# Shibodd/volume_path_tracer

Hardware: AMD Instinct MI355X
Metric: Msamples/s (whole node) + achieved HBM GB/s, wdas_cloud 1920×1080 (higher is better)
Workload: dtype f32

## Files before the change

### __graft_entry__.py

```python
from __future__ import annotations

import subprocess
import sys
from pathlib import Path

ROOT = Path(__file__).resolve().parent


def build() -> None:
    sys.path.insert(0, str(ROOT))
    from volume_path_tracer_amd import build as B

    B.build(verbose=True)
    subprocess.run(["make", "-s", "-C", str(ROOT / "oracle")], check=True)
    subprocess.run(["make", "-s", "-C", str(ROOT / "tests" / "native")], check=True)
    subprocess.run([sys.executable, "-B", "-c", "import sys; sys.path[:0] = [%r, %r]; import alpha_lib, denoise_lib, "
                    "dense_pool_lib; alpha_lib.build_lib(); denoise_lib.build_lib(); dense_pool_lib.build_program()"
                    % (str(ROOT), str(ROOT / "tests"))], check=True)
    import volume_path_tracer_amd
    from volume_path_tracer_amd import capi

    capi.lib()


def smoke() -> None:
    sys.path.insert(0, str(ROOT))
    sys.path.insert(0, str(ROOT / "tests"))
    import numpy as np
    import torch

    import oracle_lib as O
    from volume_path_tracer_amd.render import Integrator
# ... 24 lines not shown
```

### include/vpt_gpu.h

```cpp
#ifndef VPT_GPU_H
#define VPT_GPU_H

#include <stddef.h>
#include <stdint.h>

#ifdef __cplusplus
extern "C" {
#endif

#define VPT_ABI_VERSION 1

enum {
  VPT_OK = 0,
  VPT_E_INVALID = 1,
  VPT_E_HIP = 2,
  VPT_E_IO = 3,
  VPT_E_PARSE = 4,
  VPT_E_NOMEM = 5,
  VPT_E_STATE = 6
};


typedef struct vpt_camera_params {
  float position[3];
// ... 202 lines not shown
  int32_t active;
  float maximum;
} vpt_dda_row;
int vpt_dda_trace(const vpt_grid_desc* density, const float origin[3], const float direction[3], vpt_dda_row* rows,
                  int max_rows, int* n_rows);

int vpt_gpu_majorant_trace(vpt_gpu_ctx* ctx, const float origin[3], const float direction[3],
                           float* rows_host, int max_rows, int* n_rows);

enum { VPT_RNG_REFERENCE = 0, VPT_RNG_PIXEL = 1 };
int vpt_gpu_set_rng_mode(vpt_gpu_ctx* ctx, int mode);
int vpt_gpu_set_pixel_chunk(vpt_gpu_ctx* ctx, int chunk);

int vpt_gpu_set_run_skipping(vpt_gpu_ctx* ctx, int mode);
int vpt_gpu_kernel_variant(const vpt_gpu_ctx* ctx, int* has_temperature, int* run_skipping);

enum {
  VPT_ORDER_JID = 0,
  VPT_ORDER_COST_WAVE_MAJOR = 1,
  VPT_ORDER_COST_TILE_MAJOR = 2,
  VPT_ORDER_COST_TAIL = 3,
  VPT_ORDER_COST_SAME_TILE = 4
};
int vpt_gpu_set_job_order(vpt_gpu_ctx* ctx, int mode);
int vpt_gpu_set_job_order_tail(vpt_gpu_ctx* ctx, int waves);
int vpt_gpu_tile_costs(vpt_gpu_ctx* ctx, float* cost_T, uint32_t* rank_T);
int vpt_gpu_set_tile_costs(vpt_gpu_ctx* ctx, const float* cost_T);
int vpt_gpu_set_job_permutation(vpt_gpu_ctx* ctx, const uint32_t* perm, uint64_t n);

int vpt_gpu_sync(vpt_gpu_ctx* ctx);
// ... 57 lines not shown
```

### volume_path_tracer_amd/capi.py

```python
from __future__ import annotations

import ctypes as C
import os
from pathlib import Path

import numpy as np

PKG_DIR = Path(__file__).resolve().parent
LIB_DIR = PKG_DIR / "lib"
LIB_PATH = Path(os.environ["VPT_LIB"]) if os.environ.get("VPT_LIB") else LIB_DIR / "libvpt_amd.so"

VPT_OK = 0
VPT_BLACKBODY_ROWS = 500


class CameraParams(C.Structure):
    _fields_ = [("position", C.c_float * 3), ("look", C.c_float * 3), ("up", C.c_float * 3),
                ("vfov_deg", C.c_float), ("imaging_ratio", C.c_float)]


class WorkerParams(C.Structure):
    _fields_ = [("single_pixel_enabled", C.c_int32), ("use_jitter", C.c_int32),
                ("single_pixel_coord", C.c_int64 * 2),
                ("infinite_light_xyz", C.c_float * 3), ("infinite_light_multiplier", C.c_float),
# ... 256 lines not shown
    L.vpt_synth_grid.argtypes = [C.c_int, C.c_int]
    L.vpt_synth_grid.restype = gridp
    L.vpt_synth_free.argtypes = [gridp]
    L.vpt_grid_from_nanovdb.argtypes = [C.c_void_p, C.c_size_t, C.POINTER(gridp)]
    L.vpt_grid_read_nvdb.argtypes = [C.c_char_p, C.c_char_p, C.POINTER(gridp)]
    L.vpt_grid_free.argtypes = [gridp]
    L.vpt_film_to_srgb8.argtypes = [fp, C.c_int64, C.c_int64, C.POINTER(C.c_uint8)]
    L.vpt_gpu_trace_jobs.argtypes = [vp, C.c_uint64, C.c_uint64, vp, vp, C.c_uint64, C.POINTER(C.c_uint64), vp]
    L.vpt_gpu_majorant_trace.argtypes = [vp, fp, fp, fp, C.c_int, C.POINTER(C.c_int)]
    L.vpt_dda_trace.argtypes = [C.POINTER(GridDesc), fp, fp, vp, C.c_int, C.POINTER(C.c_int)]
    L.vpt_gpu_set_rng_mode.argtypes = [vp, C.c_int]
    if hasattr(L, "vpt_gpu_set_pixel_chunk"):
        L.vpt_gpu_set_pixel_chunk.argtypes = [vp, C.c_int]
    L.vpt_gpu_set_run_skipping.argtypes = [vp, C.c_int]
    L.vpt_gpu_kernel_variant.argtypes = [vp, C.POINTER(C.c_int), C.POINTER(C.c_int)]
    if hasattr(L, "vpt_gpu_set_film_order"):
        L.vpt_gpu_set_film_order.argtypes = [vp, C.c_int, C.c_uint64]
        L.vpt_gpu_film_order_info.argtypes = [vp, C.POINTER(C.c_int), C.POINTER(C.c_uint64),
                                              C.POINTER(C.c_uint64), C.POINTER(C.c_uint64)]
    if hasattr(L, "vpt_gpu_set_pool_layout"):
        L.vpt_gpu_set_pool_layout.argtypes = [vp, C.c_int]
        L.vpt_gpu_set_pool_cap.argtypes = [vp, C.c_uint64]
        L.vpt_gpu_pool_info.argtypes = [vp, C.POINTER(C.c_int), C.POINTER(C.c_int), C.POINTER(C.c_uint64),
                                        C.POINTER(C.c_uint64), C.POINTER(C.c_double)]
        L.vpt_gpu_debug_read_pool.argtypes = [vp, C.c_int, C.c_uint64, C.c_uint64, fp]
    L.vpt_gpu_set_job_order.argtypes = [vp, C.c_int]
    L.vpt_gpu_set_job_order_tail.argtypes = [vp, C.c_int]
    L.vpt_gpu_tile_costs.argtypes = [vp, fp, C.POINTER(C.c_uint32)]
    L.vpt_gpu_set_tile_costs.argtypes = [vp, fp]
    L.vpt_gpu_set_job_permutation.argtypes = [vp, C.POINTER(C.c_uint32), C.c_uint64]
# ... 63 lines not shown
```

### volume_path_tracer_amd/csrc/vpt_ctx.h

```cpp
#pragma once

#include <hip/hip_runtime.h>

#include <atomic>
#include <chrono>
#include <cstdint>
#include <mutex>
#include <string>
#include <vector>

#include "vpt_internal.h"
#include "vpt_launch.h"

#define VPT_HIP(call)                                                                                 \
  do {                                                                                                \
    hipError_t e_ = (call);                                                                           \
    if (e_ != hipSuccess)                                                                             \
      return ::vpt::set_error(VPT_E_HIP, std::string(#call " failed: ") + hipGetErrorString(e_));            \
  } while (0)

#ifndef VPT_DEFAULT_JOB_ORDER
#define VPT_DEFAULT_JOB_ORDER VPT_ORDER_COST_SAME_TILE
#endif

// ... 51 lines not shown
  uint64_t film_count = 0;
  unsigned long long* job_counter = nullptr;
  hipEvent_t slot_done[64] = {};
  bool slot_used[64] = {};
  uint32_t next_slot = 0;
  std::mutex slot_mu;
  unsigned long long* counters = nullptr;
  unsigned long long* prof = nullptr;
  vpt::DevScene* scene_dev = nullptr;
  vpt::DevScene* scene_lat_dev = nullptr;
  int lat_gate[4] = {1, 65, 1, 1};
  int lat_wave_lanes = 0;
  vpt::DevScene* scene_full_dev = nullptr;
  int full_gate[4] = {0, 0, 0, 0};
  int last_gate_set = -1;
  hipStream_t stream = nullptr;
  bool use_runs = false;
  int pixel_chunk = 0;
  int grid_blocks = 0;
  int cus = 1;
  bool grid_user = false;
  int order_mode = VPT_DEFAULT_JOB_ORDER;
  int order_tail_waves = 0;
  uint32_t* order = nullptr;
  std::vector<float> tile_cost;
  uint32_t* perm = nullptr;
  uint64_t perm_n = 0;
  std::vector<uint32_t> tile_rank;
  float* staging = nullptr;
  std::vector<vpt_gpu_feed*> feed_pool;
// ... 82 lines not shown
```

### volume_path_tracer_amd/csrc/vpt_gpu.hip

```cpp
#include <hip/hip_runtime.h>
#include <pthread.h>
#include <sched.h>
#include <unistd.h>

#include <algorithm>
#include <cmath>
#include <cstdio>
#include <cstdlib>
#include <cstring>
#include <fstream>
#include <functional>
#include <memory>
#include <atomic>
#include <mutex>
#include <chrono>
#include <string>
#include <thread>
#include <vector>

#include "vpt_ctx.h"
#include "vpt_kernels.h"
#include "vpt_denoise.h"

namespace vpt {
// ... 553 lines not shown
  } else if (feed) {
    auto kernel = temp ? vpt::vpt_integrate_kernel<true, false, false, false, false, true>
                       : ctx->use_runs ? vpt::vpt_integrate_kernel<false, false, true, false, false, true>
                                       : vpt::vpt_integrate_kernel<false, false, false, false, false, true>;
    hipLaunchKernelGGL(kernel, dim3(blocks), dim3(vpt::kBlockThreads), 0, s, env, scene, ctx->counters);
  } else {
    auto kernel = temp ? (dbg ? vpt::vpt_integrate_kernel<true, true, false> : vpt::vpt_integrate_kernel<true, false, false>)
                       : ctx->use_runs
                           ? (dbg ? vpt::vpt_integrate_kernel<false, true, true> : vpt::vpt_integrate_kernel<false, false, true>)
                           : (dbg ? vpt::vpt_integrate_kernel<false, true, false> : vpt::vpt_integrate_kernel<false, false, false>);
    if (!dbg && scene == ctx->scene_dev) scene = ctx->scene_full_dev;
    hipLaunchKernelGGL(kernel, dim3(blocks), dim3(vpt::kBlockThreads), 0, s, env, scene, ctx->counters);
  }
  ctx->last_gate_set = scene == ctx->scene_full_dev ? VPT_GATES_FULL
                       : scene == ctx->scene_lat_dev ? VPT_GATES_LATENCY : VPT_GATES_CONTEXT;
  VPT_HIP(hipGetLastError());
  const uint64_t npix = (uint64_t)ctx->scene.W * (uint64_t)ctx->scene.H;
  if (band) {
    const uint32_t chunks = (ctx->scene.tile_area + 63u) / 64u;
    const uint32_t* const list = band->list ? ctx->list_dev : nullptr;
    hipLaunchKernelGGL(ctx->m2 ? vpt::vpt_band_order_kernel<true> : vpt::vpt_band_order_kernel<false>,
                       dim3(band->tiles * chunks), dim3(64), 0, s, ctx->scene_dev, env.film, (const float*)samples,
                       band->tile_lo, band->waves, env.band_groups, band->group, list, ctx->m2);
    VPT_HIP(hipGetLastError());
    VPT_HIP(hipEventRecord(ctx->samples_done, s));
    ctx->samples_used = true;
  } else if (samples) {
    const uint64_t threads = ctx->scene.T * (uint64_t)ctx->scene.tile_area;
    hipLaunchKernelGGL(ctx->m2 ? vpt::vpt_film_order_kernel<true> : vpt::vpt_film_order_kernel<false>,
                       dim3((unsigned)((threads + 255) / 256)), dim3(256), 0, s, ctx->scene_dev, env.film,
// ... 646 lines not shown
  env.gang_target = p->target_error;
  env.gang_floor = p->abs_floor;
  env.gang_min = p->min_waves;
  env.gang_step = p->step_waves;
  env.gang_max = p->max_waves;
  uint32_t slot = 0;
  if ((rc = take_slot(ctx, s, slot))) return rc;
  env.job_counter = ctx->job_counter + 2 * slot;
  env.event_count = ctx->job_counter + 2 * slot + 1;
  const bool temp = ctx->scene.has_temperature != 0;
  auto kernel = temp ? vpt::vpt_integrate_kernel<true, false, false, false, false, false, false, true>
                     : ctx->use_runs ? vpt::vpt_integrate_kernel<false, false, true, false, false, false, false, true>
                                     : vpt::vpt_integrate_kernel<false, false, false, false, false, false, false, true>;
  hipLaunchKernelGGL(kernel, dim3(blocks), dim3(vpt::kBlockThreads), 0, s, env, ctx->scene_full_dev, ctx->counters);
  ctx->last_gate_set = VPT_GATES_FULL;
  VPT_HIP(hipGetLastError());
  ++ctx->ordered_launches;
  VPT_HIP(hipMemcpyAsync(waves_T_host, ctx->gang_waves, (size_t)T * sizeof(uint32_t), hipMemcpyDeviceToHost, s));
  VPT_HIP(hipMemcpyAsync(err_T_host, ctx->tile_err, (size_t)T * sizeof(float), hipMemcpyDeviceToHost, s));
  if ((rc = release_slot(ctx, s, slot))) return rc;
  VPT_HIP(hipStreamSynchronize(s));
  vpt_adaptive_result res{};
  res.jobs_uniform = (uint64_t)p->max_waves * T;
  uint32_t longest = p->min_waves;
  for (uint32_t t = 0; t < T; ++t) {
    res.jobs_rendered += waves_T_host[t];
    longest = std::max(longest, waves_T_host[t]);
    if (waves_T_host[t] >= p->max_waves) ++res.tiles_at_max;
    res.max_error = std::max(res.max_error, err_T_host[t]);
  }
// ... 68 lines not shown
  return VPT_OK;
}

int vpt_gpu_set_run_skipping(vpt_gpu_ctx* ctx, int mode) {
  if (!ctx || mode < -1 || mode > 1) return vpt::set_error(VPT_E_INVALID, "vpt_gpu_set_run_skipping: bad argument");
  if (mode == 1 && ctx->scene.has_temperature)
    return vpt::set_error(VPT_E_INVALID, "vpt_gpu_set_run_skipping: no run-skipping variant with a temperature grid");
  ctx->use_runs = mode < 0 ? (!ctx->scene.has_temperature && ctx->density.run_fraction >= VPT_RUNS_MIN_FRACTION) : mode == 1;
  return VPT_OK;
}

int vpt_gpu_kernel_variant(const vpt_gpu_ctx* ctx, int* has_temperature, int* run_skipping) {
  if (!ctx) return vpt::set_error(VPT_E_INVALID, "null context");
  if (has_temperature) *has_temperature = ctx->scene.has_temperature ? 1 : 0;
  if (run_skipping) *run_skipping = ctx->use_runs ? 1 : 0;
  return VPT_OK;
}

int vpt_gpu_set_pool_layout(vpt_gpu_ctx* ctx, int layout) {
  if (!ctx || layout < VPT_POOL_SPARSE || layout > VPT_POOL_AUTO)
    return vpt::set_error(VPT_E_INVALID, "vpt_gpu_set_pool_layout: bad argument");
  if (ctx->open_feeds.load() > 0) return vpt::set_error(VPT_E_STATE, "vpt_gpu_set_pool_layout: a feed of this context is open");
  if (ctx->frame_waves) return vpt::set_error(VPT_E_STATE, "vpt_gpu_set_pool_layout: a frame is open");
  int rc = ctx_device(ctx);
  if (rc) return rc;
  if ((rc = wait_ctx(ctx))) return rc;
  VPT_HIP(hipDeviceSynchronize());
  ctx->pool_policy = layout;
  rc = apply_pool_layout(ctx, layout);
  const int prc = push_scene(ctx);
// ... 459 lines not shown
```

### volume_path_tracer_amd/csrc/vpt_integrator.h

```cpp
#pragma once

#include <hip/hip_runtime.h>
#include <stdint.h>

#include "vpt_math.h"

namespace vpt {

struct RootTileDev {
  int32_t origin[3];
  float value;
  int32_t active;
  int32_t pad[3];
};

struct DevGrid {
  float mat[9], inv_mat[9], vec[3];
  float background;
  int32_t bbox_min[3], bbox_max[3];
  int32_t r8_org[3], r8_n[3];
  int32_t w8_org[3], w8_n[3];
  uint32_t w8_max;
  int32_t r128_org[3], r128_n[3];
  int32_t root_count, leaf_count;
// ... 141 lines not shown
    }
  }
}

__host__ __device__ __forceinline__ void dense_square(const DevGrid& g, int32_t a, int32_t b, int32_t c, int32_t s,
                                                      float out[4]) {
  const int32_t x = s % 9, yz = s / 9;
  const int32_t i = g.r8_org[0] + a * 8 + x, j = g.r8_org[1] + b * 8 + (yz >> 3), k = g.r8_org[2] + c * 8 + (yz & 7);
  out[0] = value_at(g, i, j, k);
  out[1] = value_at(g, i, j, k + 1);
  out[2] = value_at(g, i, j + 1, k);
  out[3] = value_at(g, i, j + 1, k + 1);
}

__host__ __device__ __forceinline__ float lerpf(float a, float b, float w) { return a + w * (b - a); }
__host__ __device__ __forceinline__ bool trilinear(const DevGrid& g, StencilCell& last, float x, float y, float z,
                                                   float& out) {
  float fi = floorf(x), fj = floorf(y), fk = floorf(z);
  float u = x - fi, v = y - fj, w = z - fk;
  int32_t i = (int32_t)fi, j = (int32_t)fj, k = (int32_t)fk;
  bool refresh = i != last.i || j != last.j || k != last.k;
  if (g.dense) {
    const int32_t a = (i - g.r8_org[0]) >> 3, b = (j - g.r8_org[1]) >> 3, c = (k - g.r8_org[2]) >> 3;
    if ((uint32_t)a < (uint32_t)g.r8_n[0] && (uint32_t)b < (uint32_t)g.r8_n[1] && (uint32_t)c < (uint32_t)g.r8_n[2]) {
      const float4* p = reinterpret_cast<const float4*>(g.dense + dense_index(mad_index(a, b, c, g.r8_n), i, j, k));
      const float4 lo = p[0], hi = p[1];
      last.i = i;
      last.j = j;
      last.k = k;
      last.code = -1;
// ... 185 lines not shown
#endif
  return q / rw;
}

enum : int32_t {
  ST_FETCH = 0,
  ST_PIXEL = 1,
  ST_RAY = 2,
  ST_SAMPLE = 3,
  ST_NEE_DONE = 4,
  ST_FINISH = 5,
  ST_DONE = 6,
  ST_SHADOW = 7,
  ST_FINISH_T = 8
};
enum : int32_t { SM_NEED_SEG = 0, SM_STEP = 1, SM_DRAW = 2, SM_EVAL = 3, SM_NONE = 4 };
enum : int32_t {
  PB_ITER = 0, PB_FETCH, PB_PIXEL, PB_RAY, PB_SAMPLE, PB_NEED_SEG, PB_STEP, PB_DRAW, PB_TRILINEAR,
  PB_EVENT, PB_SHADOW_HIT, PB_NONE, PB_NEE_DONE, PB_FINISH,
  PB_W_WALK, PB_W_EVAL, PB_W_NEE, PB_W_FIN, PB_W_RAY, PB_W_PIX, PB_W_DONE, PB_COUNT
};
enum : int32_t { PT_FETCH = 0, PT_PIXEL, PT_RAY, PT_WALK, PT_EVAL, PT_NEE, PT_FINISH, PT_SEG, PT_STEP, PT_DRAW, PT_COUNT };

enum : int32_t {
  CNT_SAMPLES = 0, CNT_DDA_STEPS, CNT_SEGMENTS, CNT_DRAWS, CNT_STENCILS, CNT_DENSITY_EVALS, CNT_TEMP_STENCILS,
  CNT_SCATTERS, CNT_SHADOW_RAYS, CNT_RNG_DRAWS, CNT_EXCHANGED, CNT_COUNT
};

struct LaneCold {
  int32_t x0, y0, pix;
  uint32_t depth;
// ... 390 lines not shown
      for (int i = 0; i < 3; ++i) lc.ro[i] = cp[i];
      if (S.li_zero) {
        lc.Tr = -1.0f;
        ln.state = ST_NEE_DONE;
      } else {
        lc.Tr = local_const(1.0f);
        ln.shadow = 1;
        ln.state = ST_SHADOW;
      }
    }
  }
  if (Debug && ev == 0) env.event(ln, VPT_EV_NULL, nullptr, nullptr, 0.0f);
  if (ev != 0) ln.sm = SM_NONE;
}

template <bool HasTemp, bool Debug, class Env>
__host__ __device__ __forceinline__ void eval_collision(ScenePtr sp, const DevScene& S, const DevGrid& G, Lane& ln, Env& env) {
  LaneCold& lc = env.cold();
  const float sigma_maj = ln.s_dmaj * S.sigma_t;
  {
    const float dt_m = -math::logf_glibc_unit(lc.y_draw, env.logf_table()) / sigma_maj;
    const float tc = ln.s_t0 + math::div_by_recip(dt_m, ln.scale, ln.rscale);
    if (!(tc < ln.s_t1)) {
      ln.sm = SM_NEED_SEG;
      return;
    }
    ln.s_t0 = tc;
  }
  env.prof(PB_TRILINEAR);
  const float t = ln.s_t0;
  float pi_x = ln.e[0] + ln.d[0] * t, pi_y = ln.e[1] + ln.d[1] * t, pi_z = ln.e[2] + ln.d[2] * t;
  float dens;
  if (Debug) env.tally(CNT_DENSITY_EVALS, 1);
  env.tally(CNT_STENCILS, trilinear(G, lc.dens_cell, pi_x, pi_y, pi_z, dens) ? 1 : 0);
  ln.sm = SM_DRAW;
  if (dens > 0.0f) {
    if (!HasTemp) {
      const bool sh = ln.shadow != 0;
      const float sigma_n = fmaxf(0.0f, sigma_maj - S.sigma_t * dens);
      const float q1 = (sh ? sigma_n : S.sigma_a * dens) / sigma_maj;
      const float tr = lc.Tr * q1;
      const bool draw = !sh || tr <= 0.05f;
      float u = 0.0f;
      if (draw) {
        u = rng_uniform(ln.rng);
        if (Debug) env.tally(CNT_RNG_DRAWS, 1);
      }
      if (!sh) {
        primary_event<HasTemp, Debug>(sp, S, G, ln, lc, env, pi_x, pi_y, pi_z, dens, q1, (S.sigma_s * dens) / sigma_maj, u);
// ... 82 lines not shown
  ln.scale = ln.rscale = ln.maj = ln.Tn = ln.T1 = ln.s_t0 = ln.s_t1 = ln.s_dmaj = 0.0f;
  ln.dim = 0;
  ln.pw = 0;
}

template <class Env, class = void>
struct env_is_gang {
  static constexpr bool value = false;
};
template <class Env>
struct env_is_gang<Env, decltype((void)Env::kGang)> {
  static constexpr bool value = Env::kGang;
};


template <bool HasTemp, bool Debug, bool Runs, class Env>
__host__ __device__ __forceinline__ void lane_iteration(ScenePtr sp, Lane& ln, Env& env) {
  env.prof(PB_ITER);
  LaneCold& lc = env.cold();
  int32_t gate_min;
  bool starving;
  {
    const DevScene S = *opaque(sp);
    gate_min = S.gate_min;
    const int32_t n_walking = env.count(ln.state == ST_SAMPLE && ln.sm != SM_EVAL);
    starving = n_walking < S.gate_idle;
  }
  auto go = [&](int32_t st) -> bool {
    const int32_t n = env.count(ln.state == st);
    return n > 0 && (starving || n >= gate_min) && ln.state == st;
  };
  auto go2 = [&](int32_t st_a, int32_t st_b) -> bool {
    const bool mine = ln.state == st_a || ln.state == st_b;
    const int32_t n = env.count(mine);
    return n > 0 && (starving || n >= gate_min) && mine;
  };

  {
    const DevScene S = *opaque(sp);
    const DevGrid& G = S.density;
    (void)G;
    if (go(ST_NEE_DONE)) {
      env.prof(PB_NEE_DONE);
      if (lc.Tr >= 0.0f) {
        float c = lc.rd[0] * S.wi[0] + (lc.rd[1] * S.wi[1] + lc.rd[2] * S.wi[2]);
        float p = hg_eval(S, c);
        float pt = p * lc.Tr;
        lc.L[0] = lc.L[0] + pt * S.Li[0];
        lc.L[1] = lc.L[1] + pt * S.Li[1];
        lc.L[2] = lc.L[2] + pt * S.Li[2];
      } else {
        lc.L[0] = lc.L[0] == 0.0f ? 0.0f : lc.L[0];
        lc.L[1] = lc.L[1] == 0.0f ? 0.0f : lc.L[1];
        lc.L[2] = lc.L[2] == 0.0f ? 0.0f : lc.L[2];
      }
      float u0 = rng_uniform(ln.rng);
      float u1 = rng_uniform(ln.rng);
      if (Debug) env.tally(CNT_RNG_DRAWS, 2);
      float nd[3];
      sample_hg(S, lc.rd, u0, u1, nd);
      for (int i = 0; i < 3; ++i) lc.rd[i] = nd[i];
      if (Debug) env.event(ln, VPT_EV_SCATTER, lc.ro, lc.rd, 0.0f);
      ++lc.depth;
      ln.shadow = 0;
      ln.state = ST_RAY;
    }
  }
  env.tick(PT_NEE);
  {
    const DevScene S = *opaque(sp);
    const DevGrid& G = S.density;
    (void)G;
    const bool fin = go2(ST_FINISH, ST_FINISH_T);
    if (fin) {
      env.prof(PB_FINISH);
      if (ln.state == ST_FINISH) {
        lc.L[0] = lc.L[0] + S.le_inf[0];
        lc.L[1] = lc.L[1] + S.le_inf[1];
        lc.L[2] = lc.L[2] + S.le_inf[2];
      }
      const int32_t rw = min(S.W - lc.x0, S.tw);
      const int32_t q = (lc.pix & kPixelMask) - 1, y = div_pix(q, rw);
      env.film_add(S, ln, lc.x0 + (q - y * rw), lc.y0 + y, rw);
// ... 134 lines not shown
        dv[1] = math::div_by_recip(dv[1], s, rs);
        dv[2] = math::div_by_recip(dv[2], s, rs);
      }
      for (int i = 0; i < 3; ++i) {
        lc.ro[i] = S.cam_pos[i];
        lc.rd[i] = dv[i];
        lc.L[i] = 0.0f;
      }
      lc.depth = 0;
      ln.shadow = 0;
      ln.state = ST_RAY;
      if (Debug) env.event(ln, VPT_EV_NEW_RAY, lc.ro, lc.rd, 0.0f);
    }
  }
  env.tick(PT_PIXEL);
  {
    const DevScene S = *opaque(sp);
    const DevGrid& G = S.density;
    (void)G;
    if (go2(ST_RAY, ST_SHADOW)) {
      env.prof(PB_RAY);
      const bool primary = ln.state == ST_RAY;
      if (primary && !(lc.depth < S.max_depth)) {
        ln.state = ST_FINISH;
      } else {
        RayDir rd;
        if (primary) {
          rd = ray_dir_setup(G, lc.rd);
        } else {
          for (int i = 0; i < 3; ++i) {
// ... 81 lines not shown
        } else {
          lc.y_draw = y;
          ln.sm = SM_EVAL;
        }
      }
      env.tick(PT_DRAW);
#if VPT_WALK_UNROLL > 1
      }
#endif
      } while (S.gate_walk > 0 && env.count(ln.state == ST_SAMPLE && ln.sm != SM_EVAL) >= S.gate_walk &&
               env.count(ln.state == ST_SAMPLE && ln.sm == SM_EVAL) < S.gate_eval);
      wave_priority(0);
    }
  }
  env.tick(PT_WALK);
  {
    const DevScene S = *opaque(sp);
    const DevGrid& G = S.density;
    (void)G;
    const int32_t n_eval = env.count(ln.state == ST_SAMPLE && ln.sm == SM_EVAL);
    const bool run_eval = n_eval > 0 && (n_eval >= S.gate_eval || env.count(ln.state == ST_SAMPLE && ln.sm != SM_EVAL) < S.gate_idle);
    if (!HasTemp && run_eval) wave_priority(kPrioEval);
    if (run_eval && ln.state == ST_SAMPLE && ln.sm == SM_EVAL) eval_collision<HasTemp, Debug>(sp, S, G, ln, env);
    if (!HasTemp) wave_priority(0);
  }
  env.tick(PT_EVAL);
}

__host__ __device__ __forceinline__ void lane_init(Lane& ln) {
  ln.state = ST_FETCH;
  ln.sm = SM_NONE;
// ... 13 lines not shown
```

### volume_path_tracer_amd/csrc/vpt_kernels.h

```cpp
#pragma once

#include <hip/hip_runtime.h>

#include "vpt_alpha.h"
#include "vpt_internal.h"
#include "vpt_launch.h"

namespace vpt {

constexpr int kCounterCount = CNT_COUNT;
#ifndef VPT_WAVES_FAST
#define VPT_WAVES_FAST 7
#endif
#ifndef VPT_WAVES_SLOW
#define VPT_WAVES_SLOW 4
#endif
#ifndef VPT_WAVES_TEMP
#define VPT_WAVES_TEMP 6
#endif
#ifndef VPT_WAVES_LAT
#define VPT_WAVES_LAT 4
#endif

__shared__ LaneCold g_lane_cold[kBlockThreads];
// ... 45 lines not shown
  uint32_t* gang_waves;
  float* gang_err;
  float gang_target, gang_floor;
  uint32_t gang_min, gang_step, gang_max;
};
typedef const __attribute__((address_space(4))) KernelArgs* ArgsPtr;
__shared__ unsigned long long g_wg_counters[kCounterCount];
#if defined(VPT_PROFILE) || defined(VPT_PROFILE_TIME)
__shared__ unsigned long long g_wg_prof[PT_COUNT + kBlockThreads / 64];
#endif
__shared__ float g_bb_lds[kBbFloats];
__shared__ uint32_t g_film_rank[kBlockThreads];
__shared__ uint32_t g_gang[kBlockThreads / 64][4];
constexpr uint32_t kGangMaxArea = 256;

template <bool RegCold, bool Feed = false, bool Band = false, bool Gang = false>
struct KernelEnvT {
  static_assert(!(RegCold && Feed), "feeds run the throughput kernels only");
  static_assert(!(Band && Feed), "band launches are no feeds");
  static_assert(!(Gang && (RegCold || Feed || Band)), "gang launches run the plain throughput kernels only");
  static constexpr bool kGang = Gang;
  __device__ __forceinline__ ArgsPtr args() const {
    ArgsPtr p = (ArgsPtr)__builtin_amdgcn_kernarg_segment_ptr();
    asm volatile("" : "+s"(p));
    return p;
  }

  __device__ __forceinline__ void tally(int32_t k, int32_t w) {
    const unsigned long long m = __builtin_amdgcn_ballot_w64(w != 0);
    if (m && __lane_id() == (uint32_t)__builtin_ctzll(m))
      atomicAdd(g_wg_counters + k, (unsigned long long)(__popcll(m) * (uint64_t)(w ? w : 1)));
  }

  __device__ __forceinline__ void prof(int32_t id) {
#ifdef VPT_PROFILE
    const unsigned long long m = __ballot(1);
// ... 498 lines not shown
#pragma unroll
      for (int q = 0; q < kXWords / 4; ++q) {
        const uint4 v = g_xchg[q * kBlockThreads + threadIdx.x];
        x[4 * q] = v.x;
        x[4 * q + 1] = v.y;
        x[4 * q + 2] = v.z;
        x[4 * q + 3] = v.w;
      }
      xchg_unpack<HasTemp>(ln, lc, x);
      env.tally(CNT_EXCHANGED, 1);
    }
    __syncthreads();
  }
}

template <bool HasTemp, bool Debug, bool Runs, bool Lat = false, bool Compact = false, bool Feed = false, bool Band = false,
          bool Gang = false>
__global__ __launch_bounds__(kBlockThreads, Compact ? 2 : (Lat ? VPT_WAVES_LAT : (Debug ? VPT_WAVES_SLOW : (HasTemp ? VPT_WAVES_TEMP : VPT_WAVES_FAST)))) void vpt_integrate_kernel(KernelArgs args, const DevScene* scene,
                                                                       unsigned long long* counters) {
  (void)args;
  if (threadIdx.x < kCounterCount) g_wg_counters[threadIdx.x] = 0;
  if (threadIdx.x < 32) g_logf_tab[threadIdx.x >> 1][threadIdx.x & 1] = math::kLogfTab[threadIdx.x >> 1][threadIdx.x & 1];
  if (HasTemp) {
    const float* bb = scene->bb;
    for (int i = threadIdx.x; i < kBbFloats; i += kBlockThreads) g_bb_lds[i] = bb[i];
  }
  __syncthreads();
#if defined(VPT_PROFILE) || defined(VPT_PROFILE_TIME)
  if (threadIdx.x < PT_COUNT) g_wg_prof[threadIdx.x] = 0;
  __syncthreads();
  if (threadIdx.x % 64 == 0) g_wg_prof[PT_COUNT + threadIdx.x / 64] = clock64();
#endif
  static_assert(!(Band && Debug), "band launches have no records or events");
  static_assert(!(Gang && (Debug || Lat || Compact || Feed || Band)), "gang launches run the plain throughput kernels only");
  if constexpr (Gang) {
    if (threadIdx.x < kBlockThreads / 64) {
      g_gang[threadIdx.x][0] = 0xffffffffu;
      g_gang[threadIdx.x][3] = 0;
    }
    __syncthreads();
  }
  KernelEnvT<Lat, Feed, Band, Gang> env;
  env.reg_cold = nullptr;
  Lane ln;
  lane_init(ln);
  LaneCold lc_reg;
  if constexpr (Lat) env.reg_cold = &lc_reg;
  cold_init(env.cold());
  const ScenePtr sp = (ScenePtr)scene;
  if constexpr (Compact) {
    static_assert(Lat && !Debug, "compaction runs in the latency kernel only");
    compact_loop<HasTemp, Runs>(sp, ln, lc_reg, env);
  } else
  while (ln.state != ST_DONE) {
    lane_iteration<HasTemp, Debug, Runs>(sp, ln, env);
    if (Feed &&
        __builtin_amdgcn_ballot_w64(ln.state == ST_FETCH && (env.cold().pix == kFeedPending ||
// ... 411 lines not shown
```

### volume_path_tracer_amd/render.py

```python
from __future__ import annotations

import ctypes as C
import threading
import time
from typing import Optional

import numpy as np

from . import capi


def ceildiv(a: int, b: int) -> int:
    return a // b + (a % b != 0)


class TileProvider:

    def __init__(self, img_size, waves: int, tile_size):
        self.img_w, self.img_h = int(img_size[0]), int(img_size[1])
        self.tile_w, self.tile_h = int(tile_size[0]), int(tile_size[1])
        self.ntx, self.nty = ceildiv(self.img_w, self.tile_w), ceildiv(self.img_h, self.tile_h)
        self.num_tiles = self.ntx * self.nty
        self.requested_waves = int(waves)
        self.max_wave_idx = 0
# ... 267 lines not shown

    def set_run_skipping(self, mode: int) -> None:
        capi.check(capi.lib().vpt_gpu_set_run_skipping(self.h, int(mode)), "vpt_gpu_set_run_skipping")

    def set_latency_kernel(self, mode: int, ungated: int = -1) -> None:
        capi.check(capi.lib().vpt_gpu_set_latency_kernel(self.h, int(mode), int(ungated)), "vpt_gpu_set_latency_kernel")

    def set_compaction(self, every: int) -> None:
        capi.check(capi.lib().vpt_gpu_set_compaction(self.h, int(every)), "vpt_gpu_set_compaction")

    def latency_kernel_info(self) -> dict:
        m, b = C.c_int(), C.c_int()
        capi.check(capi.lib().vpt_gpu_latency_kernel_info(self.h, C.byref(m), C.byref(b)), "vpt_gpu_latency_kernel_info")
        return {"mode": int(m.value), "resident_blocks_per_cu": int(b.value)}

    def kernel_variant(self) -> dict:
        t, r = C.c_int(), C.c_int()
        capi.check(capi.lib().vpt_gpu_kernel_variant(self.h, C.byref(t), C.byref(r)), "vpt_gpu_kernel_variant")
        return {"has_temperature": bool(t.value), "run_skipping": bool(r.value)}

    def set_film_order(self, mode: int, max_bytes: int = 0) -> None:
        capi.check(capi.lib().vpt_gpu_set_film_order(self.h, int(mode), int(max_bytes)), "vpt_gpu_set_film_order")

    def film_order_info(self) -> dict:
        m, b, o, a = C.c_int(), C.c_uint64(), C.c_uint64(), C.c_uint64()
        capi.check(capi.lib().vpt_gpu_film_order_info(self.h, C.byref(m), C.byref(b), C.byref(o), C.byref(a)),
                   "vpt_gpu_film_order_info")
        return {"mode": int(m.value), "buffer_bytes": int(b.value), "ordered_launches": int(o.value),
                "atomic_launches": int(a.value)}

    def set_pool_layout(self, layout: int, cap_bytes: int | None = None) -> None:
        if cap_bytes is not None:
            capi.check(capi.lib().vpt_gpu_set_pool_cap(self.h, int(cap_bytes)), "vpt_gpu_set_pool_cap")
        capi.check(capi.lib().vpt_gpu_set_pool_layout(self.h, int(layout)), "vpt_gpu_set_pool_layout")
# ... 208 lines not shown
```

Baseline: 1712.

## Split density evaluation into issue and finish phases to hide stencil load latency

In the throughput kernels without temperature, density evaluation is split in two. The first phase, at the top of each lane iteration, draws the collision distance and issues the dense 8-voxel stencil loads as two float4 reads. The second phase, after the pixel and fetch stages, does the trilinear interpolation and the event. Moving the NEE-done and later eval blocks lets the memory latency overlap with other state-machine work in the same iteration. The cost is extra live registers across the iteration (two float4s), new sub-states, and a different ordering of work between lanes, which could affect occupancy.

```diff
diff --git a/__graft_entry__.py b/__graft_entry__.py
--- a/__graft_entry__.py
+++ b/__graft_entry__.py
@@ -15,7 +15,8 @@
     subprocess.run(["make", "-s", "-C", str(ROOT / "oracle")], check=True)
     subprocess.run(["make", "-s", "-C", str(ROOT / "tests" / "native")], check=True)
     subprocess.run([sys.executable, "-B", "-c", "import sys; sys.path[:0] = [%r, %r]; import alpha_lib, denoise_lib, "
-                    "dense_pool_lib; alpha_lib.build_lib(); denoise_lib.build_lib(); dense_pool_lib.build_program()"
+                    "dense_pool_lib, eval_split_lib; alpha_lib.build_lib(); denoise_lib.build_lib(); "
+                    "dense_pool_lib.build_program(); eval_split_lib.build_lib()"
                     % (str(ROOT), str(ROOT / "tests"))], check=True)
     import volume_path_tracer_amd
     from volume_path_tracer_amd import capi
diff --git a/include/vpt_gpu.h b/include/vpt_gpu.h
--- a/include/vpt_gpu.h
+++ b/include/vpt_gpu.h
@@ -240,6 +240,7 @@
 
 int vpt_gpu_set_run_skipping(vpt_gpu_ctx* ctx, int mode);
 int vpt_gpu_kernel_variant(const vpt_gpu_ctx* ctx, int* has_temperature, int* run_skipping);
+int vpt_gpu_last_launch_variant(const vpt_gpu_ctx* ctx, int* eval_split);
 
 enum {
   VPT_ORDER_JID = 0,
diff --git a/volume_path_tracer_amd/capi.py b/volume_path_tracer_amd/capi.py
--- a/volume_path_tracer_amd/capi.py
+++ b/volume_path_tracer_amd/capi.py
@@ -294,6 +294,8 @@
         L.vpt_gpu_set_pixel_chunk.argtypes = [vp, C.c_int]
     L.vpt_gpu_set_run_skipping.argtypes = [vp, C.c_int]
     L.vpt_gpu_kernel_variant.argtypes = [vp, C.POINTER(C.c_int), C.POINTER(C.c_int)]
+    if hasattr(L, "vpt_gpu_last_launch_variant"):
+        L.vpt_gpu_last_launch_variant.argtypes = [vp, C.POINTER(C.c_int)]
     if hasattr(L, "vpt_gpu_set_film_order"):
         L.vpt_gpu_set_film_order.argtypes = [vp, C.c_int, C.c_uint64]
         L.vpt_gpu_film_order_info.argtypes = [vp, C.POINTER(C.c_int), C.POINTER(C.c_uint64),
diff --git a/volume_path_tracer_amd/csrc/vpt_ctx.h b/volume_path_tracer_amd/csrc/vpt_ctx.h
--- a/volume_path_tracer_amd/csrc/vpt_ctx.h
+++ b/volume_path_tracer_amd/csrc/vpt_ctx.h
@@ -89,6 +89,7 @@
   vpt::DevScene* scene_full_dev = nullptr;
   int full_gate[4] = {0, 0, 0, 0};
   int last_gate_set = -1;
+  int last_eval_split = -1;
   hipStream_t stream = nullptr;
   bool use_runs = false;
   int pixel_chunk = 0;
diff --git a/volume_path_tracer_amd/csrc/vpt_gpu.hip b/volume_path_tracer_amd/csrc/vpt_gpu.hip
--- a/volume_path_tracer_amd/csrc/vpt_gpu.hip
+++ b/volume_path_tracer_amd/csrc/vpt_gpu.hip
@@ -591,6 +591,7 @@
   }
   ctx->last_gate_set = scene == ctx->scene_full_dev ? VPT_GATES_FULL
                        : scene == ctx->scene_lat_dev ? VPT_GATES_LATENCY : VPT_GATES_CONTEXT;
+  ctx->last_eval_split = vpt::kernel_eval_split(temp, dbg, use_lat) ? 1 : 0;
   VPT_HIP(hipGetLastError());
   const uint64_t npix = (uint64_t)ctx->scene.W * (uint64_t)ctx->scene.H;
   if (band) {
@@ -1267,6 +1268,7 @@
                                      : vpt::vpt_integrate_kernel<false, false, false, false, false, false, false, true>;
   hipLaunchKernelGGL(kernel, dim3(blocks), dim3(vpt::kBlockThreads), 0, s, env, ctx->scene_full_dev, ctx->counters);
   ctx->last_gate_set = VPT_GATES_FULL;
+  ctx->last_eval_split = vpt::kernel_eval_split(temp, false, false) ? 1 : 0;
   VPT_HIP(hipGetLastError());
   ++ctx->ordered_launches;
   VPT_HIP(hipMemcpyAsync(waves_T_host, ctx->gang_waves, (size_t)T * sizeof(uint32_t), hipMemcpyDeviceToHost, s));
@@ -1365,6 +1367,12 @@
   if (!ctx) return vpt::set_error(VPT_E_INVALID, "null context");
   if (has_temperature) *has_temperature = ctx->scene.has_temperature ? 1 : 0;
   if (run_skipping) *run_skipping = ctx->use_runs ? 1 : 0;
+  return VPT_OK;
+}
+
+int vpt_gpu_last_launch_variant(const vpt_gpu_ctx* ctx, int* eval_split) {
+  if (!ctx) return vpt::set_error(VPT_E_INVALID, "null context");
+  if (eval_split) *eval_split = ctx->last_eval_split;
   return VPT_OK;
 }
 
diff --git a/volume_path_tracer_amd/csrc/vpt_integrator.h b/volume_path_tracer_amd/csrc/vpt_integrator.h
--- a/volume_path_tracer_amd/csrc/vpt_integrator.h
+++ b/volume_path_tracer_amd/csrc/vpt_integrator.h
@@ -179,6 +179,31 @@
 }
 
 __host__ __device__ __forceinline__ float lerpf(float a, float b, float w) { return a + w * (b - a); }
+__host__ __device__ __forceinline__ const float4* dense_stencil(const DevGrid& g, int32_t i, int32_t j, int32_t k) {
+  if (g.dense) {
+    const int32_t a = (i - g.r8_org[0]) >> 3, b = (j - g.r8_org[1]) >> 3, c = (k - g.r8_org[2]) >> 3;
+    if ((uint32_t)a < (uint32_t)g.r8_n[0] && (uint32_t)b < (uint32_t)g.r8_n[1] && (uint32_t)c < (uint32_t)g.r8_n[2])
+      return reinterpret_cast<const float4*>(g.dense + dense_index(mad_index(a, b, c, g.r8_n), i, j, k));
+  }
+  return nullptr;
+}
+__host__ __device__ __forceinline__ void lookup_stencil(const DevGrid& g, StencilCell& last, int32_t i, int32_t j, int32_t k,
+                                                        float s[8]) {
+  const int32_t dx = (i ^ last.i) | (j ^ last.j) | (k ^ last.k);
+  const bool same_leaf = last.code >= 0 && dx >= 0 && dx < 8;
+  Cell c;
+  if (same_leaf) {
+    c.code = last.code;
+    c.value = 0.0f;
+  } else {
+    c = cell_at(g, i, j, k);
+  }
+  last.i = i;
+  last.j = j;
+  last.k = k;
+  last.code = c.code;
+  fetch_stencil(g, c, i, j, k, s);
+}
 __host__ __device__ __forceinline__ bool trilinear(const DevGrid& g, StencilCell& last, float x, float y, float z,
                                                    float& out) {
   float fi = floorf(x), fj = floorf(y), fk = floorf(z);
@@ -394,7 +419,7 @@
   ST_SHADOW = 7,
   ST_FINISH_T = 8
 };
-enum : int32_t { SM_NEED_SEG = 0, SM_STEP = 1, SM_DRAW = 2, SM_EVAL = 3, SM_NONE = 4 };
+enum : int32_t { SM_NEED_SEG = 0, SM_STEP = 1, SM_DRAW = 2, SM_EVAL = 3, SM_NONE = 4, SM_FETCHED = 5, SM_FETCHED_LOOKUP = 6 };
 enum : int32_t {
   PB_ITER = 0, PB_FETCH, PB_PIXEL, PB_RAY, PB_SAMPLE, PB_NEED_SEG, PB_STEP, PB_DRAW, PB_TRILINEAR,
   PB_EVENT, PB_SHADOW_HIT, PB_NONE, PB_NEE_DONE, PB_FINISH,
@@ -815,25 +840,90 @@
   if (ev != 0) ln.sm = SM_NONE;
 }
 
+template <class Env>
+__host__ __device__ __forceinline__ bool eval_distance(Lane& ln, const LaneCold& lc, Env& env, float sigma_maj) {
+  const float dt_m = -math::logf_glibc_unit(lc.y_draw, env.logf_table()) / sigma_maj;
+  const float tc = ln.s_t0 + math::div_by_recip(dt_m, ln.scale, ln.rscale);
+  if (!(tc < ln.s_t1)) {
+    ln.sm = SM_NEED_SEG;
+    return false;
+  }
+  ln.s_t0 = tc;
+  return true;
+}
+
+template <bool HasTemp, bool Debug, class Env>
+__host__ __device__ __forceinline__ void eval_event(ScenePtr sp, const DevScene& S, const DevGrid& G, Lane& ln, LaneCold& lc, Env& env,
+                                                    float sigma_maj, float pi_x, float pi_y, float pi_z, float dens);
+
 template <bool HasTemp, bool Debug, class Env>
 __host__ __device__ __forceinline__ void eval_collision(ScenePtr sp, const DevScene& S, const DevGrid& G, Lane& ln, Env& env) {
   LaneCold& lc = env.cold();
   const float sigma_maj = ln.s_dmaj * S.sigma_t;
-  {
-    const float dt_m = -math::logf_glibc_unit(lc.y_draw, env.logf_table()) / sigma_maj;
-    const float tc = ln.s_t0 + math::div_by_recip(dt_m, ln.scale, ln.rscale);
-    if (!(tc < ln.s_t1)) {
-      ln.sm = SM_NEED_SEG;
-      return;
-    }
-    ln.s_t0 = tc;
-  }
+  if (!eval_distance(ln, lc, env, sigma_maj)) return;
   env.prof(PB_TRILINEAR);
   const float t = ln.s_t0;
   float pi_x = ln.e[0] + ln.d[0] * t, pi_y = ln.e[1] + ln.d[1] * t, pi_z = ln.e[2] + ln.d[2] * t;
   float dens;
   if (Debug) env.tally(CNT_DENSITY_EVALS, 1);
   env.tally(CNT_STENCILS, trilinear(G, lc.dens_cell, pi_x, pi_y, pi_z, dens) ? 1 : 0);
+  eval_event<HasTemp, Debug>(sp, S, G, ln, lc, env, sigma_maj, pi_x, pi_y, pi_z, dens);
+}
+
+template <bool Debug, class Env>
+__host__ __device__ __forceinline__ void eval_issue(const DevScene& S, const DevGrid& G, Lane& ln, Env& env, float4& lo, float4& hi) {
+  LaneCold& lc = env.cold();
+  if (!eval_distance(ln, lc, env, ln.s_dmaj * S.sigma_t)) return;
+  env.prof(PB_TRILINEAR);
+  const float t = ln.s_t0;
+  const float pi_x = ln.e[0] + ln.d[0] * t, pi_y = ln.e[1] + ln.d[1] * t, pi_z = ln.e[2] + ln.d[2] * t;
+  const int32_t i = (int32_t)floorf(pi_x), j = (int32_t)floorf(pi_y), k = (int32_t)floorf(pi_z);
+  if (Debug) env.tally(CNT_DENSITY_EVALS, 1);
+  ln.sm = SM_FETCHED_LOOKUP;
+  if (const float4* p = dense_stencil(G, i, j, k)) {
+    lo = p[0];
+    hi = p[1];
+    StencilCell& last = lc.dens_cell;
+    env.tally(CNT_STENCILS, (i != last.i || j != last.j || k != last.k) ? 1 : 0);
+    last.i = i;
+    last.j = j;
+    last.k = k;
+    last.code = -1;
+    ln.sm = SM_FETCHED;
+  }
+}
+
+template <bool HasTemp, bool Debug, class Env>
+__host__ __device__ __forceinline__ void eval_finish(ScenePtr sp, const DevScene& S, const DevGrid& G, Lane& ln, Env& env,
+                                                     const float4& lo, const float4& hi) {
+  LaneCold& lc = env.cold();
+  const float t = local_value(ln.s_t0);
+  const float pi_x = ln.e[0] + ln.d[0] * t, pi_y = ln.e[1] + ln.d[1] * t, pi_z = ln.e[2] + ln.d[2] * t;
+  const float fi = floorf(pi_x), fj = floorf(pi_y), fk = floorf(pi_z);
+  const float u = pi_x - fi, v = pi_y - fj, w = pi_z - fk;
+  float s[8];
+  if (ln.sm == SM_FETCHED) {
+    s[0] = lo.x;
+    s[1] = lo.y;
+    s[2] = lo.z;
+    s[3] = lo.w;
+    s[4] = hi.x;
+    s[5] = hi.y;
+    s[6] = hi.z;
+    s[7] = hi.w;
+  } else {
+    const int32_t i = (int32_t)fi, j = (int32_t)fj, k = (int32_t)fk;
+    StencilCell& last = lc.dens_cell;
+    env.tally(CNT_STENCILS, (i != last.i || j != last.j || k != last.k) ? 1 : 0);
+    lookup_stencil(G, last, i, j, k, s);
+  }
+  const float dens = lerpf(lerpf(lerpf(s[0], s[1], w), lerpf(s[2], s[3], w), v), lerpf(lerpf(s[4], s[5], w), lerpf(s[6], s[7], w), v), u);
+  eval_event<HasTemp, Debug>(sp, S, G, ln, lc, env, ln.s_dmaj * S.sigma_t, pi_x, pi_y, pi_z, dens);
+}
+
+template <bool HasTemp, bool Debug, class Env>
+__host__ __device__ __forceinline__ void eval_event(ScenePtr sp, const DevScene& S, const DevGrid& G, Lane& ln, LaneCold& lc, Env& env,
+                                                    float sigma_maj, float pi_x, float pi_y, float pi_z, float dens) {
   ln.sm = SM_DRAW;
   if (dens > 0.0f) {
     if (!HasTemp) {
@@ -946,16 +1036,67 @@
 };
 
 
+template <bool Debug, class Env>
+__host__ __device__ __forceinline__ void nee_done(const DevScene& S, Lane& ln, LaneCold& lc, Env& env) {
+  env.prof(PB_NEE_DONE);
+  if (lc.Tr >= 0.0f) {
+    float c = lc.rd[0] * S.wi[0] + (lc.rd[1] * S.wi[1] + lc.rd[2] * S.wi[2]);
+    float p = hg_eval(S, c);
+    float pt = p * lc.Tr;
+    lc.L[0] = lc.L[0] + pt * S.Li[0];
+    lc.L[1] = lc.L[1] + pt * S.Li[1];
+    lc.L[2] = lc.L[2] + pt * S.Li[2];
+  } else {
+    lc.L[0] = lc.L[0] == 0.0f ? 0.0f : lc.L[0];
+    lc.L[1] = lc.L[1] == 0.0f ? 0.0f : lc.L[1];
+    lc.L[2] = lc.L[2] == 0.0f ? 0.0f : lc.L[2];
+  }
+  float u0 = rng_uniform(ln.rng);
+  float u1 = rng_uniform(ln.rng);
+  if (Debug) env.tally(CNT_RNG_DRAWS, 2);
+  float nd[3];
+  sample_hg(S, lc.rd, u0, u1, nd);
+  for (int i = 0; i < 3; ++i) lc.rd[i] = nd[i];
+  if (Debug) env.event(ln, VPT_EV_SCATTER, lc.ro, lc.rd, 0.0f);
+  ++lc.depth;
+  ln.shadow = 0;
+  ln.state = ST_RAY;
+}
+
+template <class Env, class = void>
+struct env_eval_split {
+  static constexpr bool value = false;
+};
+template <class Env>
+struct env_eval_split<Env, decltype((void)Env::kEvalSplit)> {
+  static constexpr bool value = Env::kEvalSplit;
+};
+
 template <bool HasTemp, bool Debug, bool Runs, class Env>
 __host__ __device__ __forceinline__ void lane_iteration(ScenePtr sp, Lane& ln, Env& env) {
   env.prof(PB_ITER);
   LaneCold& lc = env.cold();
+  constexpr bool kSplit = env_eval_split<Env>::value;
+  float4 st_lo, st_hi;
+#if !defined(__HIP_DEVICE_COMPILE__)
+  st_lo = st_hi = float4{0.0f, 0.0f, 0.0f, 0.0f};
+#endif
   int32_t gate_min;
   bool starving;
   {
     const DevScene S = *opaque(sp);
     gate_min = S.gate_min;
-    const int32_t n_walking = env.count(ln.state == ST_SAMPLE && ln.sm != SM_EVAL);
+    int32_t n_walking = env.count(ln.state == ST_SAMPLE && ln.sm != SM_EVAL);
+    if constexpr (kSplit) {
+      const DevGrid& G = S.density;
+      const int32_t n_eval = env.count(ln.state == ST_SAMPLE && ln.sm == SM_EVAL);
+      const bool run_eval = n_eval > 0 && (n_eval >= S.gate_eval || n_walking < S.gate_idle);
+      if (run_eval) wave_priority(kPrioEval);
+      if (run_eval && ln.state == ST_SAMPLE && ln.sm == SM_EVAL) eval_issue<Debug>(S, G, ln, env, st_lo, st_hi);
+      wave_priority(0);
+      if (run_eval) n_walking += n_eval;
+      env.tick(PT_EVAL);
+    }
     starving = n_walking < S.gate_idle;
   }
   auto go = [&](int32_t st) -> bool {
@@ -967,38 +1108,11 @@
     const int32_t n = env.count(mine);
     return n > 0 && (starving || n >= gate_min) && mine;
   };
-
-  {
+  if constexpr (!kSplit) {
     const DevScene S = *opaque(sp);
-    const DevGrid& G = S.density;
-    (void)G;
-    if (go(ST_NEE_DONE)) {
-      env.prof(PB_NEE_DONE);
-      if (lc.Tr >= 0.0f) {
-        float c = lc.rd[0] * S.wi[0] + (lc.rd[1] * S.wi[1] + lc.rd[2] * S.wi[2]);
-        float p = hg_eval(S, c);
-        float pt = p * lc.Tr;
-        lc.L[0] = lc.L[0] + pt * S.Li[0];
-        lc.L[1] = lc.L[1] + pt * S.Li[1];
-        lc.L[2] = lc.L[2] + pt * S.Li[2];
-      } else {
-        lc.L[0] = lc.L[0] == 0.0f ? 0.0f : lc.L[0];
-        lc.L[1] = lc.L[1] == 0.0f ? 0.0f : lc.L[1];
-        lc.L[2] = lc.L[2] == 0.0f ? 0.0f : lc.L[2];
-      }
-      float u0 = rng_uniform(ln.rng);
-      float u1 = rng_uniform(ln.rng);
-      if (Debug) env.tally(CNT_RNG_DRAWS, 2);
-      float nd[3];
-      sample_hg(S, lc.rd, u0, u1, nd);
-      for (int i = 0; i < 3; ++i) lc.rd[i] = nd[i];
-      if (Debug) env.event(ln, VPT_EV_SCATTER, lc.ro, lc.rd, 0.0f);
-      ++lc.depth;
-      ln.shadow = 0;
-      ln.state = ST_RAY;
-    }
-  }
-  env.tick(PT_NEE);
+    if (go(ST_NEE_DONE)) nee_done<Debug>(S, ln, lc, env);
+  }
+  if constexpr (!kSplit) env.tick(PT_NEE);
   {
     const DevScene S = *opaque(sp);
     const DevGrid& G = S.density;
@@ -1163,6 +1277,20 @@
     }
   }
   env.tick(PT_PIXEL);
+  if constexpr (kSplit) {
+    const DevScene S = *opaque(sp);
+    const DevGrid& G = S.density;
+    const bool fetched = ln.state == ST_SAMPLE && ln.sm >= SM_FETCHED;
+    if (env.count(fetched) > 0) wave_priority(kPrioEval);
+    if (fetched) eval_finish<HasTemp, Debug>(sp, S, G, ln, env, st_lo, st_hi);
+    wave_priority(0);
+    env.tick(PT_EVAL);
+  }
+  if constexpr (kSplit) {
+    const DevScene S = *opaque(sp);
+    if (go(ST_NEE_DONE)) nee_done<Debug>(S, ln, lc, env);
+    env.tick(PT_NEE);
+  }
   {
     const DevScene S = *opaque(sp);
     const DevGrid& G = S.density;
@@ -1274,7 +1402,7 @@
     }
   }
   env.tick(PT_WALK);
-  {
+  if constexpr (!kSplit) {
     const DevScene S = *opaque(sp);
     const DevGrid& G = S.density;
     (void)G;
diff --git a/volume_path_tracer_amd/csrc/vpt_kernels.h b/volume_path_tracer_amd/csrc/vpt_kernels.h
--- a/volume_path_tracer_amd/csrc/vpt_kernels.h
+++ b/volume_path_tracer_amd/csrc/vpt_kernels.h
@@ -83,12 +83,14 @@
 __shared__ uint32_t g_gang[kBlockThreads / 64][4];
 constexpr uint32_t kGangMaxArea = 256;
 
-template <bool RegCold, bool Feed = false, bool Band = false, bool Gang = false>
+template <bool RegCold, bool Feed = false, bool Band = false, bool Gang = false, bool Split = false>
 struct KernelEnvT {
+  static_assert(!(RegCold && Split), "the latency kernels evaluate whole");
   static_assert(!(RegCold && Feed), "feeds run the throughput kernels only");
   static_assert(!(Band && Feed), "band launches are no feeds");
   static_assert(!(Gang && (RegCold || Feed || Band)), "gang launches run the plain throughput kernels only");
   static constexpr bool kGang = Gang;
+  static constexpr bool kEvalSplit = Split;
   __device__ __forceinline__ ArgsPtr args() const {
     ArgsPtr p = (ArgsPtr)__builtin_amdgcn_kernarg_segment_ptr();
     asm volatile("" : "+s"(p));
@@ -617,6 +619,8 @@
   }
 }
 
+constexpr bool kernel_eval_split(bool has_temp, bool debug, bool lat) { return !has_temp && !debug && !lat; }
+
 template <bool HasTemp, bool Debug, bool Runs, bool Lat = false, bool Compact = false, bool Feed = false, bool Band = false,
           bool Gang = false>
 __global__ __launch_bounds__(kBlockThreads, Compact ? 2 : (Lat ? VPT_WAVES_LAT : (Debug ? VPT_WAVES_SLOW : (HasTemp ? VPT_WAVES_TEMP : VPT_WAVES_FAST)))) void vpt_integrate_kernel(KernelArgs args, const DevScene* scene,
@@ -643,7 +647,7 @@
     }
     __syncthreads();
   }
-  KernelEnvT<Lat, Feed, Band, Gang> env;
+  KernelEnvT<Lat, Feed, Band, Gang, kernel_eval_split(HasTemp, Debug, Lat)> env;
   env.reg_cold = nullptr;
   Lane ln;
   lane_init(ln);
diff --git a/volume_path_tracer_amd/render.py b/volume_path_tracer_amd/render.py
--- a/volume_path_tracer_amd/render.py
+++ b/volume_path_tracer_amd/render.py
@@ -305,10 +305,15 @@
         capi.check(capi.lib().vpt_gpu_latency_kernel_info(self.h, C.byref(m), C.byref(b)), "vpt_gpu_latency_kernel_info")
         return {"mode": int(m.value), "resident_blocks_per_cu": int(b.value)}
 
-    def kernel_variant(self) -> dict:
+    def kernel_variant(self, last_launch: bool = False) -> dict:
         t, r = C.c_int(), C.c_int()
         capi.check(capi.lib().vpt_gpu_kernel_variant(self.h, C.byref(t), C.byref(r)), "vpt_gpu_kernel_variant")
-        return {"has_temperature": bool(t.value), "run_skipping": bool(r.value)}
+        kv = {"has_temperature": bool(t.value), "run_skipping": bool(r.value)}
+        if last_launch:
+            e = C.c_int()
+            capi.check(capi.lib().vpt_gpu_last_launch_variant(self.h, C.byref(e)), "vpt_gpu_last_launch_variant")
+            kv["eval_split"] = None if e.value < 0 else bool(e.value)
+        return kv
 
     def set_film_order(self, mode: int, max_bytes: int = 0) -> None:
         capi.check(capi.lib().vpt_gpu_set_film_order(self.h, int(mode), int(max_bytes)), "vpt_gpu_set_film_order")
```

New measurement: 1736, median of 6. 1.01x the previous value.
